# tictacmenthe/F2CNN

Measured on AMD Instinct MI355X. Metric: audio-seconds/sec through filterbank+envelope (HIP, 1 MI355X per rank); the +CNN figure of BASELINE's metric is value_with_cnn / blocks.cfg4, higher is better.
Workload: dtype f64 filter state + f64 utterance FFT + f32 row FFT; 1 GPU; cfg3: filterbank + Hilbert envelope + 50 Hz LPF in one call (f32 FFT), batch of 1000 x 1 s utterances per GPU, 128 channels, ENV1 (float64) out; channels=128, lpf_hz=50, launch_batch=1000, outputs_resident_in_hbm=True, parallelism=utterance-sharded x1, no collective, utterances_sent_back_by_the_accuracy_guard=0

## Files before the change

### f2cnn_amd/csrc/f2_api.hip

```cpp
#include "f2_internal.h"

char g_f2_err[512] = {0};

int f2_fail(f2_ctx* ctx, int code, const char* fmt, ...) {
    char* dst = ctx ? ctx->err : g_f2_err;
    va_list ap;
    va_start(ap, fmt);
    vsnprintf(dst, 512, fmt, ap);
    va_end(ap);
    return code;
}

int f2_reserve(f2_ctx* ctx, f2_scratch& s, size_t bytes) {
    if (bytes <= s.bytes) return F2_OK;
    if (s.ptr) {
        F2_HIP(ctx, hipStreamSynchronize(ctx->stream));
        F2_HIP(ctx, hipFree(s.ptr));
        s.ptr = nullptr;
        s.bytes = 0;
    }
    size_t want = (bytes + 255) & ~size_t(255);
    hipError_t e = hipMalloc(&s.ptr, want);
    if (e != hipSuccess) {
        s.ptr = nullptr;
// ... 220 lines not shown
    (void)hipStreamSynchronize(ctx->stream);
    f2_scratch* all[] = {&ctx->coefs, &ctx->offsets, &ctx->stage_in, &ctx->stage_out, &ctx->stage_aux,
                         &ctx->work,  &ctx->work2,   &ctx->xbuf,      &ctx->flags,    &ctx->gather_log, &ctx->dense_in,
                         &ctx->stamps, &ctx->noise_wave, &ctx->noise_meta, &ctx->acc_meta, &ctx->score_meta};
    for (f2_scratch* s : all)
        if (s->ptr) (void)hipFree(s->ptr);
    for (auto& v : ctx->prof)
        for (auto& pr : v) {
            (void)hipEventDestroy(pr.first);
            (void)hipEventDestroy(pr.second);
        }
    for (hipEvent_t e : ctx->prof_pool) (void)hipEventDestroy(e);
    for (auto& prec : ctx->tw)
        for (f2_scratch& s : prec)
            if (s.ptr) (void)hipFree(s.ptr);
    for (auto& prec : ctx->tw_large)
        for (f2_scratch& s : prec)
            if (s.ptr) (void)hipFree(s.ptr);
    for (f2_scratch& s : ctx->tw_p3)
        if (s.ptr) (void)hipFree(s.ptr);
    for (f2_scratch& s : ctx->tw_fl)
        if (s.ptr) (void)hipFree(s.ptr);
    for (f2_scratch& s : ctx->tw_split)
        if (s.ptr) (void)hipFree(s.ptr);
    for (f2_scratch* sc : {&ctx->tw_pair[0], &ctx->tw_pair[1], &ctx->pair_list[0], &ctx->pair_list[1]})
        if (sc->ptr) (void)hipFree(sc->ptr);
    if (ctx->work3.ptr) (void)hipFree(ctx->work3.ptr);
    if (ctx->k1_states.ptr) (void)hipFree(ctx->k1_states.ptr);
    if (ctx->k1_mtab.ptr) (void)hipFree(ctx->k1_mtab.ptr);
    if (ctx->k1_order.ptr) (void)hipFree(ctx->k1_order.ptr);
    if (ctx->handoff.ptr) (void)hipFree(ctx->handoff.ptr);
    if (ctx->handoff_off.ptr) (void)hipFree(ctx->handoff_off.ptr);
    for (auto& t : ctx->spec_tabs)
        for (f2_scratch* sc : {&t.hu, &t.e, &t.lgroup, &t.e64})
            if (sc->ptr) (void)hipFree(sc->ptr);
    for (f2_scratch* sc : {&ctx->spec_x, &ctx->spec_rho, &ctx->spec_xpart, &ctx->spec_meta, &ctx->spec_uflag, &ctx->spec_lptab})
        if (sc->ptr) (void)hipFree(sc->ptr);
    for (auto& prec : ctx->tw_sp)
        for (f2_scratch& sc : prec)
            if (sc.ptr) (void)hipFree(sc.ptr);
    for (auto& sp : ctx->up_inflight) (void)hipEventDestroy(sp.done);
    for (auto& b : ctx->up_big) {
        if (b.ptr) (void)hipHostFree(b.ptr);
        (void)hipEventDestroy(b.done);
    }
    if (ctx->up_ring) (void)hipHostFree(ctx->up_ring);
    if (ctx->host_flags) (void)hipHostFree(ctx->host_flags);
    if (ctx->own_stream && ctx->stream) (void)hipStreamDestroy(ctx->stream);
    delete ctx;
    return F2_OK;
}

int f2_ctx_synchronize(f2_ctx* ctx) {
    F2_CHECK(nullptr, ctx, F2_ERR_INVALID, "ctx is NULL");
    F2_HIP(ctx, hipStreamSynchronize(ctx->stream));
    return F2_OK;
}

int f2_ctx_set_stream(f2_ctx* ctx, void* hip_stream) {
    F2_CHECK(nullptr, ctx, F2_ERR_INVALID, "ctx is NULL");
    F2_HIP(ctx, hipStreamSynchronize(ctx->stream));
    if (ctx->own_stream && ctx->stream) F2_HIP(ctx, hipStreamDestroy(ctx->stream));
    if (hip_stream) {
        ctx->stream = (hipStream_t)hip_stream;
        ctx->own_stream = false;
    } else {
        F2_HIP(ctx, hipStreamCreateWithFlags(&ctx->stream, hipStreamNonBlocking));
        ctx->own_stream = true;
    }
// ... 523 lines not shown
```

### f2cnn_amd/csrc/f2_internal.h

```cpp
#pragma once
#include <hip/hip_runtime.h>

#include <cstdarg>
#include <cstdint>
#include <cstdio>
#include <cstring>
#include <mutex>
#include <string>
#include <utility>
#include <vector>

#include "../../include/f2cnn_hip.h"

struct f2_scratch {
    void* ptr = nullptr;
    size_t bytes = 0;
};

struct f2_spec_tables {
    int log2h = 0, C = 0;
    std::vector<double> coefs;
    int64_t tpitch = 0;
    f2_scratch hu, e, lgroup, e64;
};
#define F2_SPECTRAL_MIN_LOG2H 12
#define F2_SPECTRAL_MAX_LOG2H 15

struct f2_ctx {
    int device = 0;
    hipStream_t stream = nullptr;
    bool own_stream = true;
    int num_cus = 0;
    char err[512] = {0};
    f2_scratch coefs;
    f2_scratch offsets;
    f2_scratch stage_in;
    f2_scratch stage_out;
    f2_scratch stage_aux;
    f2_scratch work;
    f2_scratch work2;
    f2_scratch xbuf;
    f2_scratch dense_in;
    f2_scratch noise_wave;
    f2_scratch noise_meta;
    f2_scratch acc_meta;
    f2_scratch score_meta;
    f2_scratch gather_log;
    f2_scratch tw[2][16];
    f2_scratch tw_fl[16];
    f2_scratch tw_p3[2];
    f2_scratch tw_large[2][24];
    f2_scratch tw_split[24];
    std::vector<int> pair_list_host[2];
    f2_scratch tw_pair[2], pair_list[2];
    f2_scratch work3;
    f2_scratch handoff, handoff_off;
    std::vector<int64_t> handoff_off_host;
    f2_scratch k1_states, k1_mtab;
    f2_scratch k1_order;
    int k1_mtab_L = 0;
    std::vector<double> k1_mtab_coefs;
    std::vector<int64_t> offsets_host;
    std::vector<double> coefs_host;
    bool prof_on = false;
    struct prof_span {
        hipEvent_t first, second;
        bool closed;
    };
    std::vector<prof_span> prof[F2_K_COUNT];
    std::vector<hipEvent_t> prof_pool;
    std::vector<f2_spec_tables> spec_tabs;
    f2_scratch spec_x, spec_rho;
    f2_scratch spec_xpart;
    f2_scratch spec_meta, spec_uflag;
    f2_scratch spec_gdump;
    size_t spec_gdump_rows = 0;
    std::vector<int> spec_meta_host;
    int spec_coefs_ok = -1;
    int spec_min_pad = 64;
    size_t spec_last_B = 0;
    f2_scratch tw_sp[2][16];
    f2_scratch spec_lptab;
    double spec_lptab_a1 = 0.0;
    int spec_lptab_nt = 0;
    int opt_spectral = 1;
    int opt_spectral_min_rows = 4096;
    float opt_spectral_tol = 4e-6f;
    int opt_spectral_min_pad = -1;
    int opt_spectral_guard_dump = 0;
    int opt_k1_split = -1;
    int opt_k1_queue = -1;
    int opt_k1_qwaves = 0;
    int opt_env_pair = 1;
    int opt_cnn_f16x3 = 1;
    int opt_cnn_ws = 1;
    int opt_cnn_ws_dense = 1;
    int opt_gather_blocked = 1;
    int opt_env_plan4 = 0;
    char* up_ring = nullptr;
    size_t up_cap = 0, up_head = 0;
    struct up_span {
        size_t begin, end;
        hipEvent_t done;
    };
// ... 139 lines not shown
                             int nutt, int log2h, int C, int lpf, double b0, double a1, const float* d_x32,
                             const int64_t* d_x32_off, const int* d_uflag = nullptr);
bool f2_envelope_pair_supports(int log2h, int precision);
int f2_launch_envelope_pair(f2_ctx* ctx, const double* d_gfb, double* d_env, const int64_t* d_offsets,
                            const int64_t* h_offsets, const int* utts, int nutt, int log2h, int C, int lpf, double b0,
                            double a1, const float* d_x32, const int64_t* d_x32_off, const int64_t* h_x32_off,
                            const int* d_uflag = nullptr);
#define F2_MAX_LOG2M_LARGE 22
int f2_launch_envelope_large(f2_ctx* ctx, const double* d_x, double* d_y, int64_t n, int C, int lpf, double b0,
                             double a1, int precision);

static inline int f2_log2_ceil(int64_t n) {
    int k = 0;
    while ((int64_t(1) << k) < n) ++k;
    return k;
}

struct f2_handoff {
    bool f32 = false;
    float* d_x32 = nullptr;
    const int64_t* d_x32_off = nullptr;
    const int64_t* h_x32_off = nullptr;
};
int f2_plan_handoff(f2_ctx* ctx, const int64_t* h_offsets, int B, int C, int precision, bool want_gfb, f2_handoff* plan);
int f2_envelopes_device(f2_ctx* ctx, const void* d_wave, int wave_dtype, const int64_t* h_offsets, int B, int C, int lpf,
                        double cutoff_hz, int fft_precision, double* d_env, double* d_gfb, bool spectral);
int f2_launch_filterbank(f2_ctx* ctx, const void* d_wave, int wave_dtype, const int64_t* d_offsets,
                         const int64_t* h_offsets, const double* d_coefs, int B, int C, double* d_gfb,
                         const f2_handoff* handoff = nullptr, const int* d_uflag = nullptr, const int* h_flag0 = nullptr);
int f2_launch_envelope(f2_ctx* ctx, const double* d_gfb, const int64_t* d_offsets, const int64_t* h_offsets,
                       int B, int C, int lpf, double cutoff_hz, int precision, double* d_env,
                       const f2_handoff* handoff = nullptr, const int* d_uflag = nullptr, const int* h_flag0 = nullptr);
bool f2_spectral_supports_len(int64_t n, int min_pad);
bool f2_spectral_supports_coefs(const std::vector<double>& coefs, int C, std::vector<int>* Lgroup, int* min_pad);
int f2_launch_spectral(f2_ctx* ctx, const void* d_wave, int wave_dtype, const int64_t* d_offsets, const double* d_coefs,
                       int C, const int* d_ulist, int nutt, int64_t min_n , int log2h, int lpf,
                       double cutoff_hz, double* d_env, int* d_uflag);
int f2_launch_gather(f2_ctx* ctx, const double* d_env, int C, int64_t N, const int64_t* d_centers,
                     int64_t first_center, int64_t n_windows, int radius, int step, int normalize, float* d_out, int* d_flag);
int f2_launch_gather_ragged(f2_ctx* ctx, const double* d_env, int C, const int64_t* d_offsets, const int64_t* d_centers,
                            const int* d_win_utt, int64_t n_windows, int radius, int step, int normalize, float* d_out,
                            int* d_flag);
int f2_upload_windows(f2_ctx* ctx, const int64_t* centers, const int* win_utt, int64_t n_windows, const int64_t** d_centers,
                      const int** d_win_utt);
struct f2_win_seg {
    int utt;
    int64_t first, count;
};
int f2_launch_gather_strided(f2_ctx* ctx, const double* d_env, int C, const int64_t* d_offsets, const int64_t* h_offsets,
                             const f2_win_seg* segs, int nseg, int radius, int step, int hop, float* d_out, int* d_flag);
bool f2_gather_strided_blocked(const f2_ctx* ctx, int C, int step, int hop);
int64_t f2_gather_strided_columns(int64_t count, int radius, int step, int hop);
struct f2_cnn_route {
    bool split = false, ws = false, ws_dense = false;
};
f2_cnn_route f2_cnn_capability(const f2_cnn* cnn);
f2_cnn_route f2_cnn_call_route(const f2_ctx* ctx, const f2_cnn* cnn, bool have_scale_set);
bool f2_cnn_ws_supported(int rows, int channels);
bool f2_dense1_ws_takes(int K, int64_t n);
int f2_launch_dense1_ws(f2_ctx* ctx, const f2_cnn* cnn, const f2_scale_set* S, const float* a4, int64_t n, int K, float* a5);
int f2_launch_cnn_ws(f2_ctx* ctx, const f2_cnn* cnn, const f2_scale_set* S, const float* d_x, int64_t n, void* a2s, float* a4);
int f2_launch_cnn(f2_ctx* ctx, const f2_cnn* cnn, const f2_scale_set* S, f2_cnn_route route, const float* d_x, int64_t n, float* d_ws,
                  float* d_scores, uint8_t* d_labels);
int f2_launch_cnn_convs(f2_ctx* ctx, const f2_cnn* cnn, const f2_scale_set* S, f2_cnn_route route, const float* d_x, int64_t n,
                        float* d_ws, float* a4);
int f2_launch_cnn_dense(f2_ctx* ctx, const f2_cnn* cnn, const f2_scale_set* S, f2_cnn_route route, const float* a4, int64_t n, float* a5,
                        float* d_scores, uint8_t* d_labels);
// ... 17 lines not shown
```

### f2cnn_amd/csrc/f2_spectral.hip

```cpp
#define f2fft f2fft_sp
#undef F2_PLAN13_PASSES
#define F2_PLAN13_PASSES 4
#include <algorithm>
#include <cmath>
#include <complex>
#include <thread>

#include "f2_fft_lds.h"

using namespace f2fft;

namespace {

typedef float f2_f4 __attribute__((ext_vector_type(4)));
constexpr int SPEC_GB = 16;

constexpr int KS_CGROUP = 32;
constexpr int KS_CGROUP_LONG = 8;
constexpr int KS_STORE_AUX = 2;
typedef unsigned int f2_u4 __attribute__((ext_vector_type(4)));
typedef unsigned int f2_u2 __attribute__((ext_vector_type(2)));
__device__ __forceinline__ __amdgpu_buffer_rsrc_t row_buffer(double* y, int n) {
    return __builtin_amdgcn_make_buffer_rsrc(y, 0, n * 8, 0x00020000);
}
// ... 642 lines not shown
    if (tid == 0) {
        const cpx<double> z0 = lds[cpad(0)];
        if constexpr (LOGD == 0) {
            Xo[0] = {(float)(z0.re + z0.im), 0.f};
            Xo[H] = {(float)(z0.re - z0.im), 0.f};
        } else {
            Xp[0] = {z0.re + z0.im, 0.0};
            Xp[H] = {z0.re - z0.im, 0.0};
        }
    }
}

template <int LOG2HS, int LOGD>
__global__ __launch_bounds__(256) void k_spectrum_combine(const cpx<double>* __restrict__ Xpart, const cpx<double>* __restrict__ e64,
                                                          cpx<float>* __restrict__ X, int64_t xpitch) {
    constexpr int D = 1 << LOGD, HS = 1 << LOG2HS, H = D * HS, M = 2 * H;
    const int ul = blockIdx.y;
    const int k = blockIdx.x * 256 + threadIdx.x;
    if (k > H) return;
    const int kk = k & (2 * HS - 1);
    double re = 0.0, im = 0.0;
#pragma unroll
    for (int ph = 0; ph < D; ++ph) {
        const cpx<double>* __restrict__ Xp = Xpart + ((size_t)ul * D + ph) * (HS + 1);
        cpx<double> xp = kk <= HS ? Xp[kk] : Xp[2 * HS - kk];
        if (kk > HS) xp.im = -xp.im;
        const cpx<double> w = e64[(ph * k) & (M - 1)];
        re += xp.re * w.re - xp.im * w.im;
        im += xp.re * w.im + xp.im * w.re;
    }
    X[(size_t)ul * xpitch + k] = {(float)re, (float)im};
}

constexpr int TAIL_TB = 32;
constexpr int TAIL_WAVES = 4;

template <typename WaveT>
__global__ __launch_bounds__((64 * TAIL_WAVES)) void k_tail_state(const WaveT* __restrict__ wave, const int64_t* __restrict__ offsets,
                                                                const double* __restrict__ coefs, int C, int groups,
                                                                const int* __restrict__ ulist, int nutt,
                                                                const int* __restrict__ Lgroup, float* __restrict__ rho,
                                                                double two_over_m) {
    __shared__ double xss[TAIL_WAVES][TAIL_TB];
    const int lane = threadIdx.x & 63;
    const int wid = __builtin_amdgcn_readfirstlane(threadIdx.x >> 6);
    const int unit = blockIdx.x * TAIL_WAVES + wid;
    if (unit >= nutt * groups) return;
    const int ul = unit / groups, g = unit - ul * groups;
    const int b = ulist[ul];
    const int64_t off = offsets[b];
    const int64_t N = offsets[b + 1] - off;
    const int cc = g * 64 + lane;
    const int c = min(cc, C - 1);
    const double* k = coefs + (size_t)c * 10;
    const double rB0 = 1.0 / k[6];
    const double b0 = k[0] * rB0, a1 = k[7] * rB0, a2 = k[8] * rB0;
    const double c1 = k[1] / k[0], c2 = k[2] / k[0], c3 = k[3] / k[0], c4 = k[4] / k[0];
    const double scale = (b0 * b0) * (b0 * b0) / k[9] * two_over_m;
    double* xs = xss[wid];
    const WaveT* w = wave + off;
    const int64_t L = min((int64_t)Lgroup[g], N);
    const int64_t nblk = (L + TAIL_TB - 1) / TAIL_TB;
    const int64_t t_begin = N - nblk * TAIL_TB;
    double z10 = 0, z11 = 0, z20 = 0, z21 = 0, z30 = 0, z31 = 0, z40 = 0, z41 = 0;
    auto sample = [&](int64_t t) { return (lane < TAIL_TB && t >= 0 && t < N) ? (double)w[t] : 0.0; };
    double xnext = sample(t_begin + lane);
    for (int64_t t0 = t_begin; t0 < N; t0 += TAIL_TB) {
        if (lane < TAIL_TB) xs[lane] = xnext;
        xnext = sample(t0 + TAIL_TB + lane);
        __builtin_amdgcn_fence(__ATOMIC_RELEASE, "wavefront");
        __builtin_amdgcn_wave_barrier();
        __builtin_amdgcn_fence(__ATOMIC_ACQUIRE, "wavefront");
        double p1 = 0, p2 = 0, p3 = 0;
#pragma unroll
        for (int s2 = 0; s2 < TAIL_TB + 3; ++s2) {
            double n1 = 0, n2 = 0, n3 = 0;
            if (s2 < TAIL_TB) {
                const double wv = fma(-a1, z10, fma(-a2, z11, xs[s2]));
                n1 = fma(c1, z10, wv);
                z11 = z10;
                z10 = wv;
            }
            if (s2 >= 1 && s2 - 1 < TAIL_TB) {
                const double wv = fma(-a1, z20, fma(-a2, z21, p1));
                n2 = fma(c2, z20, wv);
                z21 = z20;
                z20 = wv;
            }
            if (s2 >= 2 && s2 - 2 < TAIL_TB) {
                const double wv = fma(-a1, z30, fma(-a2, z31, p2));
                n3 = fma(c3, z30, wv);
                z31 = z30;
                z30 = wv;
            }
            if (s2 >= 3) {
                const double wv = fma(-a1, z40, fma(-a2, z41, p3));
                z41 = z40;
                z40 = wv;
            }
            p1 = n1;
            p2 = n2;
            p3 = n3;
        }
        __builtin_amdgcn_fence(__ATOMIC_RELEASE, "wavefront");
        __builtin_amdgcn_wave_barrier();
        __builtin_amdgcn_fence(__ATOMIC_ACQUIRE, "wavefront");
    }
    const double ia2 = 1.0 / a2;
    const double R10 = (a1 - c1) * z10 + a2 * z11, R11 = a2 * z10 + c1 * a2 * z11;
    const double R20 = (a1 - c2) * z20 + a2 * z21, R21 = a2 * z20 + c2 * a2 * z21;
    const double R30 = (a1 - c3) * z30 + a2 * z31, R31 = a2 * z30 + c3 * a2 * z31;
    const double R40 = (a1 - c4) * z40 + a2 * z41, R41 = a2 * z40 + c4 * a2 * z41;
    double d0[2], d1[2], d2[2], d3[2];
    d3[0] = R40;
    d3[1] = R41;
    {
        const double p0 = R30, p1q = R31 + c4 * R30, p2q = c4 * R31;
        const double q = p2q * ia2;
        d2[0] = p0 - q;
        d2[1] = p1q - q * a1;
        d3[0] += q;
    }
    {
        const double s0 = 1.0, s1 = c4 + c3, s2 = c4 * c3;
        double p0 = s0 * R20, p1q = s0 * R21 + s1 * R20, p2q = s1 * R21 + s2 * R20, p3q = s2 * R21;
        const double q1 = p3q * ia2;
        p2q -= q1 * a1;
        p1q -= q1;
        const double q0 = p2q * ia2;
        p1q -= q0 * a1;
        p0 -= q0;
        d1[0] = p0;
        d1[1] = p1q;
        d2[0] += q0;
        d2[1] += q1;
    }
    {
        const double s0 = 1.0, s1 = c4 + c3, s2 = c4 * c3;
        const double t0 = s0, t1 = s1 + c2 * s0, t2 = s2 + c2 * s1, t3 = c2 * s2;
        double p0 = t0 * R10, p1q = t0 * R11 + t1 * R10, p2q = t1 * R11 + t2 * R10, p3q = t2 * R11 + t3 * R10, p4q = t3 * R11;
        const double q2 = p4q * ia2;
        p3q -= q2 * a1;
        p2q -= q2;
        const double q1 = p3q * ia2;
        p2q -= q1 * a1;
        p1q -= q1;
        const double q0 = p2q * ia2;
        p1q -= q0 * a1;
        p0 -= q0;
        d0[0] = p0;
        d0[1] = p1q;
        const double qq = q2 * ia2;
        d1[0] += q0 - qq;
        d1[1] += q1 - qq * a1;
        d2[0] += qq;
    }
    if (cc < C) {
        float* r = rho + ((size_t)ul * C + cc) * 8;
        typedef float f4 __attribute__((ext_vector_type(4)));
        *reinterpret_cast<f4*>(r) = f4{(float)(d0[0] * scale), (float)(d0[1] * scale), (float)(d1[0] * scale), (float)(d1[1] * scale)};
        *reinterpret_cast<f4*>(r + 4) = f4{(float)(d2[0] * scale), (float)(d2[1] * scale), (float)(d3[0] * scale), (float)(d3[1] * scale)};
    }
}

__global__ __launch_bounds__(256) void k_spectral_tables(const double* __restrict__ coefs, int C, int H, int64_t tpitch,
                                                         f2_f4* __restrict__ hu, cpx<float>* __restrict__ e,
                                                         cpx<double>* __restrict__ e64) {
    const int M = 2 * H;
    const int64_t q = (int64_t)blockIdx.x * 256 + threadIdx.x;
    const int c = blockIdx.y;
    double sn, cs;
    sincospi(2.0 * (double)q / (double)M, &sn, &cs);
    const double wr = cs, wi = -sn;
    if (c == C) {
        if (q < M) {
            e[q] = {(float)wr, (float)wi};
            if (e64) e64[q] = {wr, wi};
        }
        return;
    }
    if (q >= tpitch) return;
    f2_f4 out = {0.f, 0.f, 0.f, 0.f};
    if (q <= H) {
        const double* k = coefs + (size_t)c * 10;
        const double rB0 = 1.0 / k[6];
        const double b0 = k[0] * rB0, a1 = k[7] * rB0, a2 = k[8] * rB0;
        const double s = (b0 * b0) * (b0 * b0) / k[9] * (2.0 / M);
        const double w2r = wr * wr - wi * wi, w2i = 2.0 * wr * wi;
        const double dr = 1.0 + a1 * wr + a2 * w2r, di = a1 * wi + a2 * w2i;
        const double dn = 1.0 / (dr * dr + di * di);
        const double ur = dr * dn, ui = -di * dn;
        double hr = s, hi = 0.0;
#pragma unroll
        for (int m = 0; m < 4; ++m) {
            const double cm = k[1 + m] / k[0];
            const double nr = 1.0 + cm * wr, ni = cm * wi;
            const double tr = nr * ur - ni * ui, ti = nr * ui + ni * ur;
            const double xr = hr * tr - hi * ti, xi = hr * ti + hi * tr;
            hr = xr;
            hi = xi;
        }
        out = {(float)hr, (float)hi, (float)ur, (float)ui};
    }
    hu[(size_t)c * tpitch + q] = out;
}

int64_t ringing_length(double a1, double a2, double tol, int64_t limit) {
    if (!(a2 > 1e-3 && a2 < 1.0) || a1 * a1 >= 4.0 * a2) return 0;
    const double lr = 0.5 * std::log(a2);
    const double np = std::max(1.0, -3.0 / lr);
    const double target = std::log(tol) + 3.0 * std::log(np) + np * lr;
    double lo = np, hi = np;
    while (3.0 * std::log(hi) + hi * lr > target) {
        hi *= 2;
        if (hi > (double)limit) return 0;
    }
    for (int it = 0; it < 60; ++it) {
        const double mid = 0.5 * (lo + hi);
        if (3.0 * std::log(mid) + mid * lr > target) lo = mid;
        else hi = mid;
    }
    return (int64_t)std::ceil(hi) + 64;
}

}

bool f2_spectral_supports_len(int64_t n, int min_pad) {
    if (n < 2) return false;
    const int log2h = f2_log2_ceil(n) - 1;
    if (log2h < F2_SPECTRAL_MIN_LOG2H || log2h > F2_SPECTRAL_MAX_LOG2H) return false;
    return (int64_t(2) << log2h) - n >= std::max(64, min_pad);
}

bool f2_spectral_supports_coefs(const std::vector<double>& coefs, int C, std::vector<int>* Lgroup, int* min_pad) {
    if (coefs.size() != (size_t)C * 10 || C <= 0) return false;
    const int groups = (C + 63) / 64;
    if (Lgroup) Lgroup->assign((size_t)groups, 0);
    double peak = 0.0;
    for (int c = 0; c < C; ++c) {
        const double* k = &coefs[(size_t)c * 10];
        if (k[5] != 0.0 || k[0] == 0.0 || k[6] == 0.0 || k[9] == 0.0) return false;
        for (int q = 0; q < 10; ++q)
            if (!std::isfinite(k[q])) return false;
        const int64_t L = ringing_length(k[7] / k[6], k[8] / k[6], 1e-8, int64_t(1) << 17);
        if (L <= 0) return false;
        if (Lgroup) (*Lgroup)[(size_t)c / 64] = std::max((*Lgroup)[(size_t)c / 64], (int)L);
        peak = std::max(peak, 3.0 / (-0.5 * std::log(k[8] / k[6])));
    }
    if (min_pad) *min_pad = ((int)std::ceil(1.1 * peak) + 31) / 32 * 32;
    return true;
}

static int spectral_tables(f2_ctx* ctx, const double* d_coefs, int C, int log2h, f2_spec_tables** out) {
    for (auto& t : ctx->spec_tabs)
        if (t.log2h == log2h && t.C == C && t.coefs == ctx->coefs_host) {
            *out = &t;
            return F2_OK;
        }
    if (ctx->spec_tabs.size() >= 6) {
        F2_HIP(ctx, hipStreamSynchronize(ctx->stream));
        for (f2_scratch* s : {&ctx->spec_tabs.front().hu, &ctx->spec_tabs.front().e, &ctx->spec_tabs.front().lgroup,
                              &ctx->spec_tabs.front().e64})
            if (s->ptr) (void)hipFree(s->ptr);
        ctx->spec_tabs.erase(ctx->spec_tabs.begin());
    }
    f2_spec_tables t;
    t.log2h = log2h;
    t.C = C;
    t.coefs = ctx->coefs_host;
    std::vector<int> Lg;
    if (!f2_spectral_supports_coefs(t.coefs, C, &Lg, nullptr)) return f2_fail(ctx, F2_ERR_INVALID, "coefficient table not eligible");
    const int H = 1 << log2h, M = 2 * H;
    t.tpitch = H + 8;
    F2_TRY(f2_reserve(ctx, t.hu, sizeof(float) * 4 * (size_t)C * (size_t)t.tpitch));
    F2_TRY(f2_reserve(ctx, t.e, sizeof(float) * 2 * (size_t)M));
    F2_TRY(f2_reserve(ctx, t.lgroup, sizeof(int) * Lg.size()));
    if (log2h > 13) F2_TRY(f2_reserve(ctx, t.e64, sizeof(double) * 2 * (size_t)M));
    hipLaunchKernelGGL(k_spectral_tables, dim3((unsigned)((M + 255) / 256), (unsigned)(C + 1)), dim3(256), 0, ctx->stream, d_coefs, C, H,
                       t.tpitch, (f2_f4*)t.hu.ptr, (cpx<float>*)t.e.ptr, (cpx<double>*)t.e64.ptr);
    F2_HIP(ctx, hipGetLastError());
    F2_TRY(f2_upload_async(ctx, t.lgroup.ptr, Lg.data(), sizeof(int) * Lg.size()));
    ctx->spec_tabs.push_back(std::move(t));
    *out = &ctx->spec_tabs.back();
    return F2_OK;
}

static int lowpass_table(f2_ctx* ctx, double a1, double b0, int nt, int sp, LowpassConsts* K, const f2_f4** d_tab) {
    const long double q = -(long double)a1;
    K->qf = (float)q;
    K->b0f = (float)b0;
    K->g1 = (float)powl(q, sp);
    K->g2 = (float)powl(q, 2 * sp);
    K->g4 = (float)powl(q, 4 * sp);
    K->g8 = (float)powl(q, 8 * sp);
    K->gw = (double)powl(q, 64 * sp);
    K->gblk = (double)powl(q, sp * nt);
    f2_scratch& slot = ctx->spec_lptab;
    double& slot_a1 = ctx->spec_lptab_a1;
    *d_tab = (const f2_f4*)slot.ptr;
    constexpr int TMAX = 1024;
    if (slot.ptr && slot_a1 == a1) return F2_OK;
    std::vector<float> tab((size_t)TMAX * 4);
    for (int t = 0; t < TMAX; ++t) {
        const int lane = t & 63;
        tab[4 * (size_t)t] = (float)powl(q, sp * (lane + 1));
        tab[4 * (size_t)t + 1] = (float)powl(q, sp * t);
        tab[4 * (size_t)t + 2] = (float)powl(q, sp * ((lane & 15) + 1));
        tab[4 * (size_t)t + 3] = (float)powl(q, sp * ((lane & 31) + 1));
    }
    F2_TRY(f2_reserve(ctx, slot, sizeof(float) * tab.size()));
    F2_TRY(f2_upload_async(ctx, slot.ptr, tab.data(), sizeof(float) * tab.size()));
    slot_a1 = a1;
    *d_tab = (const f2_f4*)slot.ptr;
    return F2_OK;
}

template <typename WaveT, int LOG2H>
static int launch_group(f2_ctx* ctx, const WaveT* d_wave, const int64_t* d_offsets, const double* d_coefs, int C,
                        const int* d_ulist, int nutt, int64_t min_n, int lpf, double b0, double a1, double* d_env, int* d_uflag,
                        float tol, cpx<float>* d_X, float* d_rho) {
    constexpr int H = 1 << LOG2H, M = 2 * H;
    f2_spec_tables* tab = nullptr;
    F2_TRY(spectral_tables(ctx, d_coefs, C, LOG2H, &tab));
    constexpr int LOGD = LOG2H > 13 ? LOG2H - 13 : 0, LOG2HS = LOG2H - LOGD;
    constexpr int FFTLOG = LOG2H == 15 ? 14 : LOG2H;
    F2_TRY(ensure_twiddles<double>(ctx, LOG2HS, ctx->tw_sp[1][LOG2HS]));
    F2_TRY(ensure_twiddles<float>(ctx, FFTLOG, ctx->tw_sp[0][FFTLOG]));
    const int64_t xpitch = H + 8;
    const int groups = (C + 63) / 64;
    F2_TRY(f2_prof_begin(ctx, F2_K_SPECTRUM));
    cpx<double>* d_part = nullptr;
    if constexpr (LOGD > 0) {
        F2_TRY(f2_reserve(ctx, ctx->spec_xpart, sizeof(double) * 2 * ((size_t)(1 << LOG2HS) + 1) * (size_t)nutt << LOGD));
        d_part = (cpx<double>*)ctx->spec_xpart.ptr;
    }
    hipLaunchKernelGGL((k_utterance_spectrum<WaveT, LOG2HS, LOGD>), dim3((unsigned)nutt << LOGD), dim3(threads_for<double, LOG2HS>()),
                       0, ctx->stream, d_wave, d_offsets, d_ulist, d_X, xpitch, d_part,
                       (const cpx<double>*)ctx->tw_sp[1][LOG2HS].ptr);
    F2_HIP(ctx, hipGetLastError());
    if constexpr (LOGD > 0) {
        hipLaunchKernelGGL((k_spectrum_combine<LOG2HS, LOGD>), dim3((unsigned)((H + 256) / 256), (unsigned)nutt), dim3(256), 0,
                           ctx->stream, (const cpx<double>*)d_part, (const cpx<double>*)tab->e64.ptr, d_X, xpitch);
        F2_HIP(ctx, hipGetLastError());
    }
    F2_TRY(f2_prof_end(ctx, F2_K_SPECTRUM));
    F2_TRY(f2_prof_begin(ctx, F2_K_TAIL));
    const int units = nutt * groups;
    hipLaunchKernelGGL((k_tail_state<WaveT>), dim3((unsigned)((units + TAIL_WAVES - 1) / TAIL_WAVES)), dim3(64 * TAIL_WAVES), 0,
                       ctx->stream, d_wave, d_offsets, d_coefs, C, groups, d_ulist, nutt, (const int*)tab->lgroup.ptr, d_rho,
                       2.0 / M);
    F2_HIP(ctx, hipGetLastError());
    F2_TRY(f2_prof_end(ctx, F2_K_TAIL));
    SpecParams P;
    P.xpitch = xpitch;
    P.tpitch = tab->tpitch;
    P.env = d_env;
    P.uflag = d_uflag;
    P.C = C;
    P.nutt = nutt;
    P.lpf = lpf;
    const f2_f4* d_lptab = nullptr;
    F2_TRY(lowpass_table(ctx, a1, b0, threads_for<float, FFTLOG>(), 2, &P.lp, &d_lptab));
    P.tol = tol;
    P.gdump = ctx->opt_spectral_guard_dump ? (float*)ctx->spec_gdump.ptr : nullptr;
    P.stamps = nullptr;
#ifdef F2_STAMPS
    F2_TRY(f2_stamps_buffer(ctx, (size_t)nutt * C, 8, &P.stamps));
#endif
    F2_TRY(f2_prof_begin(ctx, F2_K_FUSED));
    if constexpr (LOG2H == 15)
        hipLaunchKernelGGL(k_spectral_envelope_long, dim3((unsigned)((size_t)nutt * C)), dim3(threads_for<float, FFTLOG>()), 0,
                           ctx->stream, P, (const cpx<float>*)d_X, (const f2_f4*)tab->hu.ptr, (const cpx<float>*)tab->e.ptr,
                           (const float*)d_rho, d_offsets, d_ulist, d_lptab, (const cpx<float>*)ctx->tw_sp[0][FFTLOG].ptr);
    else if (min_n >= 15 * (M / 16))
        hipLaunchKernelGGL((k_spectral_envelope<FFTLOG, true>), dim3((unsigned)((size_t)nutt * C)), dim3(threads_for<float, FFTLOG>()), 0,
                           ctx->stream, P, (const cpx<float>*)d_X, (const f2_f4*)tab->hu.ptr, (const cpx<float>*)tab->e.ptr,
                           (const float*)d_rho, d_offsets, d_ulist, d_lptab, (const cpx<float>*)ctx->tw_sp[0][FFTLOG].ptr);
    else
        hipLaunchKernelGGL((k_spectral_envelope<FFTLOG, false>), dim3((unsigned)((size_t)nutt * C)), dim3(threads_for<float, FFTLOG>()), 0,
                           ctx->stream, P, (const cpx<float>*)d_X, (const f2_f4*)tab->hu.ptr, (const cpx<float>*)tab->e.ptr,
                           (const float*)d_rho, d_offsets, d_ulist, d_lptab, (const cpx<float>*)ctx->tw_sp[0][FFTLOG].ptr);
    F2_HIP(ctx, hipGetLastError());
    F2_TRY(f2_prof_end(ctx, F2_K_FUSED));
// ... 39 lines not shown
```

Before: 203,800 audio-seconds/s.

## Compute spectral tail state as a matrix product with precomputed impulse-response table

The per-channel sequential IIR recurrence that computed each utterance's tail filter state is replaced by a linear map. The host precomputes, for each channel pair, the impulse-response contribution of each tail sample to the 8 state digits and uploads it as a table. The kernel then evaluates the tail state with f64 MFMA (16x16x4) over tiles of 64 utterances, using buffer loads into LDS and a cross-wave reduction. This removes the serial per-sample dependency chain and uses matrix units, at the cost of a cached table of up to 64 MB and of a fixed length cap that could change accuracy for slowly decaying channels.

After: 205,000 audio-seconds/s (median of 6 runs). No clear change (+0.6%).

```diff
diff --git a/f2cnn_amd/csrc/f2_api.hip b/f2cnn_amd/csrc/f2_api.hip
--- a/f2cnn_amd/csrc/f2_api.hip
+++ b/f2cnn_amd/csrc/f2_api.hip
@@ -276,9 +276,9 @@
     if (ctx->handoff.ptr) (void)hipFree(ctx->handoff.ptr);
     if (ctx->handoff_off.ptr) (void)hipFree(ctx->handoff_off.ptr);
     for (auto& t : ctx->spec_tabs)
-        for (f2_scratch* sc : {&t.hu, &t.e, &t.lgroup, &t.e64})
+        for (f2_scratch* sc : {&t.hu, &t.e, &t.e64})
             if (sc->ptr) (void)hipFree(sc->ptr);
-    for (f2_scratch* sc : {&ctx->spec_x, &ctx->spec_rho, &ctx->spec_xpart, &ctx->spec_meta, &ctx->spec_uflag, &ctx->spec_lptab})
+    for (f2_scratch* sc : {&ctx->spec_tail.g, &ctx->spec_tail.meta, &ctx->spec_x, &ctx->spec_rho, &ctx->spec_xpart, &ctx->spec_meta, &ctx->spec_uflag, &ctx->spec_lptab})
         if (sc->ptr) (void)hipFree(sc->ptr);
     for (auto& prec : ctx->tw_sp)
         for (f2_scratch& sc : prec)
diff --git a/f2cnn_amd/csrc/f2_internal.h b/f2cnn_amd/csrc/f2_internal.h
--- a/f2cnn_amd/csrc/f2_internal.h
+++ b/f2cnn_amd/csrc/f2_internal.h
@@ -21,7 +21,12 @@
     int log2h = 0, C = 0;
     std::vector<double> coefs;
     int64_t tpitch = 0;
-    f2_scratch hu, e, lgroup, e64;
+    f2_scratch hu, e, e64;
+};
+struct f2_tail_table {
+    int C = 0;
+    std::vector<double> coefs;
+    f2_scratch g, meta;
 };
 #define F2_SPECTRAL_MIN_LOG2H 12
 #define F2_SPECTRAL_MAX_LOG2H 15
@@ -70,6 +75,7 @@
     std::vector<prof_span> prof[F2_K_COUNT];
     std::vector<hipEvent_t> prof_pool;
     std::vector<f2_spec_tables> spec_tabs;
+    f2_tail_table spec_tail;
     f2_scratch spec_x, spec_rho;
     f2_scratch spec_xpart;
     f2_scratch spec_meta, spec_uflag;
@@ -275,7 +281,7 @@
                        int B, int C, int lpf, double cutoff_hz, int precision, double* d_env,
                        const f2_handoff* handoff = nullptr, const int* d_uflag = nullptr, const int* h_flag0 = nullptr);
 bool f2_spectral_supports_len(int64_t n, int min_pad);
-bool f2_spectral_supports_coefs(const std::vector<double>& coefs, int C, std::vector<int>* Lgroup, int* min_pad);
+bool f2_spectral_supports_coefs(const std::vector<double>& coefs, int C, std::vector<int>* Lchan, int* min_pad);
 int f2_launch_spectral(f2_ctx* ctx, const void* d_wave, int wave_dtype, const int64_t* d_offsets, const double* d_coefs,
                        int C, const int* d_ulist, int nutt, int64_t min_n , int log2h, int lpf,
                        double cutoff_hz, double* d_env, int* d_uflag);
diff --git a/f2cnn_amd/csrc/f2_spectral.hip b/f2cnn_amd/csrc/f2_spectral.hip
--- a/f2cnn_amd/csrc/f2_spectral.hip
+++ b/f2cnn_amd/csrc/f2_spectral.hip
@@ -698,80 +698,216 @@
     X[(size_t)ul * xpitch + k] = {(float)re, (float)im};
 }
 
-constexpr int TAIL_TB = 32;
 constexpr int TAIL_WAVES = 4;
+constexpr int TAIL_UNIT = 8;
+constexpr int TAIL_XP = 65;
+constexpr int64_t TAIL_LMAX = 65472;
+constexpr size_t TAIL_TABLE_CAP = size_t(64) << 20;
+typedef double f2_d4v __attribute__((ext_vector_type(4)));
+
+template <typename WaveT>
+struct tail_stage {
+    typedef double type;
+    typedef double raw;
+    static constexpr int TS = 32;
+    static __device__ __forceinline__ raw load(__amdgpu_buffer_rsrc_t r, int byte_off) {
+        return __builtin_bit_cast(double, __builtin_amdgcn_raw_buffer_load_b64(r, byte_off, 0, 0));
+    }
+};
+template <>
+struct tail_stage<int16_t> {
+    typedef float type;
+    typedef int16_t raw;
+    static constexpr int TS = 64;
+    static __device__ __forceinline__ raw load(__amdgpu_buffer_rsrc_t r, int byte_off) {
+        return (int16_t)__builtin_amdgcn_raw_buffer_load_b16(r, byte_off, 0, 0);
+    }
+};
 
 template <typename WaveT>
 __global__ __launch_bounds__((64 * TAIL_WAVES)) void k_tail_state(const WaveT* __restrict__ wave, const int64_t* __restrict__ offsets,
-                                                                const double* __restrict__ coefs, int C, int groups,
-                                                                const int* __restrict__ ulist, int nutt,
-                                                                const int* __restrict__ Lgroup, float* __restrict__ rho,
-                                                                double two_over_m) {
-    __shared__ double xss[TAIL_WAVES][TAIL_TB];
+                                                                const double* __restrict__ coefs, int C,
+                                                                const int* __restrict__ ulist, int nutt, int ntiles,
+                                                                const double* __restrict__ G, const int* __restrict__ gmeta,
+                                                                float* __restrict__ rho, double two_over_m) {
+    typedef tail_stage<WaveT> stage;
+    typedef typename stage::type StageT;
+    typedef double __attribute__((may_alias)) double_alias;
+    constexpr int TS = stage::TS;
+    static_assert(sizeof(StageT) * TS * TAIL_XP >= sizeof(double) * 16 * 64, "the partial sums reuse a wave's staging area");
+    static_assert(TAIL_WAVES == 4 && TAIL_UNIT % 8 == 0, "four rows per instruction, two instructions per round of the loop");
+    __shared__ __attribute__((aligned(16))) StageT xss[TAIL_WAVES][TS * TAIL_XP];
     const int lane = threadIdx.x & 63;
     const int wid = __builtin_amdgcn_readfirstlane(threadIdx.x >> 6);
-    const int unit = blockIdx.x * TAIL_WAVES + wid;
-    if (unit >= nutt * groups) return;
-    const int ul = unit / groups, g = unit - ul * groups;
-    const int b = ulist[ul];
-    const int64_t off = offsets[b];
-    const int64_t N = offsets[b + 1] - off;
-    const int cc = g * 64 + lane;
-    const int c = min(cc, C - 1);
-    const double* k = coefs + (size_t)c * 10;
-    const double rB0 = 1.0 / k[6];
-    const double b0 = k[0] * rB0, a1 = k[7] * rB0, a2 = k[8] * rB0;
-    const double c1 = k[1] / k[0], c2 = k[2] / k[0], c3 = k[3] / k[0], c4 = k[4] / k[0];
-    const double scale = (b0 * b0) * (b0 * b0) / k[9] * two_over_m;
-    double* xs = xss[wid];
-    const WaveT* w = wave + off;
-    const int64_t L = min((int64_t)Lgroup[g], N);
-    const int64_t nblk = (L + TAIL_TB - 1) / TAIL_TB;
-    const int64_t t_begin = N - nblk * TAIL_TB;
-    double z10 = 0, z11 = 0, z20 = 0, z21 = 0, z30 = 0, z31 = 0, z40 = 0, z41 = 0;
-    auto sample = [&](int64_t t) { return (lane < TAIL_TB && t >= 0 && t < N) ? (double)w[t] : 0.0; };
-    double xnext = sample(t_begin + lane);
-    for (int64_t t0 = t_begin; t0 < N; t0 += TAIL_TB) {
-        if (lane < TAIL_TB) xs[lane] = xnext;
-        xnext = sample(t0 + TAIL_TB + lane);
+    const int npairs = (C + 1) / 2;
+    const int p = npairs - 1 - (int)(blockIdx.x / (unsigned)ntiles);
+    const int u0 = (int)(blockIdx.x % (unsigned)ntiles) * 64;
+    const int per = gmeta[2 * p + 1] / TAIL_WAVES;
+    const int t_begin = wid * per;
+    const double* __restrict__ g = G + ((size_t)gmeta[2 * p] + (size_t)t_begin) * 16 + lane;
+    StageT* xs = xss[wid];
+    typename stage::raw xr[64];
+    unsigned base_lo, base_hi;
+    int nbytes;
+    {
+        const int b = ulist[min(u0 + lane, nutt - 1)];
+        const int64_t off = offsets[b];
+        const unsigned long long a = (unsigned long long)(wave + off);
+        base_lo = (unsigned)a;
+        base_hi = (unsigned)(a >> 32);
+        nbytes = u0 + lane < nutt ? (int)(offsets[b + 1] - off) * (int)sizeof(WaveT) : 0;
+    }
+    auto fetch = [&](int tb) {
+        const int tbytes = (tb + lane + 1) * (int)sizeof(WaveT);
+#pragma unroll
+        for (int j = 0; j < 64; ++j) {
+            const unsigned long long a = ((unsigned long long)(unsigned)__builtin_amdgcn_readlane((int)base_hi, j) << 32) |
+                                         (unsigned)__builtin_amdgcn_readlane((int)base_lo, j);
+            const int nb = __builtin_amdgcn_readlane(nbytes, j);
+            const __amdgpu_buffer_rsrc_t r = __builtin_amdgcn_make_buffer_rsrc((WaveT*)a, 0, nb, 0x00020000);
+            xr[j] = stage::load(r, nb - tbytes);
+        }
+    };
+    double bn[TS / 4];
+    auto fetch_rows = [&](int s) {
+        const int cnt = min(TS, per - s * TS);
+        const double* __restrict__ gs = g + (size_t)s * (TS * 16);
+#pragma unroll
+        for (int q = 0; q < TS / 4; q += 2) {
+            bn[q] = bn[q + 1] = 0.0;
+            if (4 * q < cnt) {
+                bn[q] = gs[q * 64];
+                bn[q + 1] = gs[(q + 1) * 64];
+            }
+        }
+    };
+    const f2_d4v zero = {0.0, 0.0, 0.0, 0.0};
+    const double first = lane < 16 ? 1.0 : 0.0, index = lane < 16 ? (double)lane : 0.0;
+    const f2_d4v rowv = __builtin_amdgcn_mfma_f64_16x16x4f64(index, first, zero, 0, 0, 0);
+    const f2_d4v colv = __builtin_amdgcn_mfma_f64_16x16x4f64(first, index, zero, 0, 0, 0);
+    f2_d4v acc[4] = {zero, zero, zero, zero};
+    const int xrow = (lane >> 4) * TAIL_XP + (lane & 15);
+    const int nblk = (per + TS - 1) / TS;
+    fetch(t_begin);
+    fetch_rows(0);
+    for (int s = 0; s < nblk; ++s) {
+        if (TS == 64 || lane < TS) {
+#pragma unroll
+            for (int j = 0; j < 64; ++j) xs[lane * TAIL_XP + j] = (StageT)xr[j];
+        }
+        double bc[TS / 4];
+#pragma unroll
+        for (int q = 0; q < TS / 4; ++q) {
+            bc[q] = bn[q];
+            asm volatile("" : "+v"(bc[q]));
+        }
         __builtin_amdgcn_fence(__ATOMIC_RELEASE, "wavefront");
         __builtin_amdgcn_wave_barrier();
         __builtin_amdgcn_fence(__ATOMIC_ACQUIRE, "wavefront");
-        double p1 = 0, p2 = 0, p3 = 0;
-#pragma unroll
-        for (int s2 = 0; s2 < TAIL_TB + 3; ++s2) {
-            double n1 = 0, n2 = 0, n3 = 0;
-            if (s2 < TAIL_TB) {
-                const double wv = fma(-a1, z10, fma(-a2, z11, xs[s2]));
-                n1 = fma(c1, z10, wv);
-                z11 = z10;
-                z10 = wv;
+        if (s + 1 < nblk) {
+            fetch(t_begin + (s + 1) * TS);
+            fetch_rows(s + 1);
+        }
+#pragma unroll
+        for (int q = 0; q < TS / 4; ++q)
+#pragma unroll
+            for (int m = 0; m < 4; ++m) {
+                const double a = (double)xs[4 * q * TAIL_XP + xrow + 16 * m];
+                acc[m] = __builtin_amdgcn_mfma_f64_16x16x4f64(a, bc[q], acc[m], 0, 0, 0);
             }
-            if (s2 >= 1 && s2 - 1 < TAIL_TB) {
-                const double wv = fma(-a1, z20, fma(-a2, z21, p1));
-                n2 = fma(c2, z20, wv);
-                z21 = z20;
-                z20 = wv;
-            }
-            if (s2 >= 2 && s2 - 2 < TAIL_TB) {
-                const double wv = fma(-a1, z30, fma(-a2, z31, p2));
-                n3 = fma(c3, z30, wv);
-                z31 = z30;
-                z30 = wv;
-            }
-            if (s2 >= 3) {
-                const double wv = fma(-a1, z40, fma(-a2, z41, p3));
-                z41 = z40;
-                z40 = wv;
-            }
-            p1 = n1;
-            p2 = n2;
-            p3 = n3;
-        }
         __builtin_amdgcn_fence(__ATOMIC_RELEASE, "wavefront");
         __builtin_amdgcn_wave_barrier();
         __builtin_amdgcn_fence(__ATOMIC_ACQUIRE, "wavefront");
     }
+    double_alias* red = reinterpret_cast<double_alias*>(xs);
+#pragma unroll
+    for (int r = 0; r < 4; ++r) {
+        const int row = (int)rowv[r] & 15, col = (int)colv[r] & 15;
+#pragma unroll
+        for (int m = 0; m < 4; ++m) red[col * 64 + 16 * m + row] = acc[m][r];
+    }
+    __syncthreads();
+    double sum[4] = {0.0, 0.0, 0.0, 0.0};
+#pragma unroll
+    for (int w = 0; w < TAIL_WAVES; ++w) {
+        const double_alias* rw = reinterpret_cast<const double_alias*>(xss[w]);
+#pragma unroll
+        for (int q = 0; q < 4; ++q) sum[q] += rw[(4 * wid + q) * 64 + lane];
+    }
+    const int c = 2 * p + (wid >> 1);
+    const int ul = u0 + lane;
+    if (ul < nutt && c < C) {
+        const double* k = coefs + (size_t)c * 10;
+        const double b0 = k[0] * (1.0 / k[6]);
+        const double scale = (b0 * b0) * (b0 * b0) / k[9] * two_over_m;
+        typedef float f4v __attribute__((ext_vector_type(4)));
+        *reinterpret_cast<f4v*>(rho + ((size_t)ul * C + c) * 8 + 4 * (wid & 1)) =
+            f4v{(float)(sum[0] * scale), (float)(sum[1] * scale), (float)(sum[2] * scale), (float)(sum[3] * scale)};
+    }
+}
+
+__global__ __launch_bounds__(256) void k_spectral_tables(const double* __restrict__ coefs, int C, int H, int64_t tpitch,
+                                                         f2_f4* __restrict__ hu, cpx<float>* __restrict__ e,
+                                                         cpx<double>* __restrict__ e64) {
+    const int M = 2 * H;
+    const int64_t q = (int64_t)blockIdx.x * 256 + threadIdx.x;
+    const int c = blockIdx.y;
+    double sn, cs;
+    sincospi(2.0 * (double)q / (double)M, &sn, &cs);
+    const double wr = cs, wi = -sn;
+    if (c == C) {
+        if (q < M) {
+            e[q] = {(float)wr, (float)wi};
+            if (e64) e64[q] = {wr, wi};
+        }
+        return;
+    }
+    if (q >= tpitch) return;
+    f2_f4 out = {0.f, 0.f, 0.f, 0.f};
+    if (q <= H) {
+        const double* k = coefs + (size_t)c * 10;
+        const double rB0 = 1.0 / k[6];
+        const double b0 = k[0] * rB0, a1 = k[7] * rB0, a2 = k[8] * rB0;
+        const double s = (b0 * b0) * (b0 * b0) / k[9] * (2.0 / M);
+        const double w2r = wr * wr - wi * wi, w2i = 2.0 * wr * wi;
+        const double dr = 1.0 + a1 * wr + a2 * w2r, di = a1 * wi + a2 * w2i;
+        const double dn = 1.0 / (dr * dr + di * di);
+        const double ur = dr * dn, ui = -di * dn;
+        double hr = s, hi = 0.0;
+#pragma unroll
+        for (int m = 0; m < 4; ++m) {
+            const double cm = k[1 + m] / k[0];
+            const double nr = 1.0 + cm * wr, ni = cm * wi;
+            const double tr = nr * ur - ni * ui, ti = nr * ui + ni * ur;
+            const double xr = hr * tr - hi * ti, xi = hr * ti + hi * tr;
+            hr = xr;
+            hi = xi;
+        }
+        out = {(float)hr, (float)hi, (float)ur, (float)ui};
+    }
+    hu[(size_t)c * tpitch + q] = out;
+}
+
+int64_t ringing_length(double a1, double a2, double tol, int64_t limit) {
+    if (!(a2 > 1e-3 && a2 < 1.0) || a1 * a1 >= 4.0 * a2) return 0;
+    const double lr = 0.5 * std::log(a2);
+    const double np = std::max(1.0, -3.0 / lr);
+    const double target = std::log(tol) + 3.0 * std::log(np) + np * lr;
+    double lo = np, hi = np;
+    while (3.0 * std::log(hi) + hi * lr > target) {
+        hi *= 2;
+        if (hi > (double)limit) return 0;
+    }
+    for (int it = 0; it < 60; ++it) {
+        const double mid = 0.5 * (lo + hi);
+        if (3.0 * std::log(mid) + mid * lr > target) lo = mid;
+        else hi = mid;
+    }
+    return (int64_t)std::ceil(hi) + 64;
+}
+
+void tail_digits(double a1, double a2, double c1, double c2, double c3, double c4, double z10, double z11, double z20,
+                 double z21, double z30, double z31, double z40, double z41, double* d) {
     const double ia2 = 1.0 / a2;
     const double R10 = (a1 - c1) * z10 + a2 * z11, R11 = a2 * z10 + c1 * a2 * z11;
     const double R20 = (a1 - c2) * z20 + a2 * z21, R21 = a2 * z20 + c2 * a2 * z21;
@@ -821,72 +957,50 @@
         d1[1] += q1 - qq * a1;
         d2[0] += qq;
     }
-    if (cc < C) {
-        float* r = rho + ((size_t)ul * C + cc) * 8;
-        typedef float f4 __attribute__((ext_vector_type(4)));
-        *reinterpret_cast<f4*>(r) = f4{(float)(d0[0] * scale), (float)(d0[1] * scale), (float)(d1[0] * scale), (float)(d1[1] * scale)};
-        *reinterpret_cast<f4*>(r + 4) = f4{(float)(d2[0] * scale), (float)(d2[1] * scale), (float)(d3[0] * scale), (float)(d3[1] * scale)};
-    }
-}
-
-__global__ __launch_bounds__(256) void k_spectral_tables(const double* __restrict__ coefs, int C, int H, int64_t tpitch,
-                                                         f2_f4* __restrict__ hu, cpx<float>* __restrict__ e,
-                                                         cpx<double>* __restrict__ e64) {
-    const int M = 2 * H;
-    const int64_t q = (int64_t)blockIdx.x * 256 + threadIdx.x;
-    const int c = blockIdx.y;
-    double sn, cs;
-    sincospi(2.0 * (double)q / (double)M, &sn, &cs);
-    const double wr = cs, wi = -sn;
-    if (c == C) {
-        if (q < M) {
-            e[q] = {(float)wr, (float)wi};
-            if (e64) e64[q] = {wr, wi};
-        }
-        return;
-    }
-    if (q >= tpitch) return;
-    f2_f4 out = {0.f, 0.f, 0.f, 0.f};
-    if (q <= H) {
-        const double* k = coefs + (size_t)c * 10;
+    d[0] = d0[0], d[1] = d0[1], d[2] = d1[0], d[3] = d1[1], d[4] = d2[0], d[5] = d2[1], d[6] = d3[0], d[7] = d3[1];
+}
+
+int64_t tail_rows(int64_t L) {
+    constexpr int64_t Q = TAIL_WAVES * TAIL_UNIT;
+    return (L + Q - 1) / Q * Q;
+}
+
+int tail_pair_length(const std::vector<int>& Lc, int p) {
+    const size_t c = 2 * (size_t)p;
+    return c + 1 < Lc.size() ? std::max(Lc[c], Lc[c + 1]) : Lc[c];
+}
+
+void tail_table_host(const std::vector<double>& coefs, int C, const std::vector<int>& Lc, std::vector<double>* G,
+                     std::vector<int>* meta) {
+    const int npairs = (C + 1) / 2;
+    meta->assign((size_t)2 * npairs, 0);
+    int64_t rows = 0;
+    for (int p = 0; p < npairs; ++p) {
+        (*meta)[2 * (size_t)p] = (int)rows;
+        (*meta)[2 * (size_t)p + 1] = (int)tail_rows(tail_pair_length(Lc, p));
+        rows += tail_rows(tail_pair_length(Lc, p));
+    }
+    G->assign((size_t)rows * 16, 0.0);
+    for (int c = 0; c < C; ++c) {
+        const double* k = &coefs[(size_t)c * 10];
         const double rB0 = 1.0 / k[6];
-        const double b0 = k[0] * rB0, a1 = k[7] * rB0, a2 = k[8] * rB0;
-        const double s = (b0 * b0) * (b0 * b0) / k[9] * (2.0 / M);
-        const double w2r = wr * wr - wi * wi, w2i = 2.0 * wr * wi;
-        const double dr = 1.0 + a1 * wr + a2 * w2r, di = a1 * wi + a2 * w2i;
-        const double dn = 1.0 / (dr * dr + di * di);
-        const double ur = dr * dn, ui = -di * dn;
-        double hr = s, hi = 0.0;
-#pragma unroll
-        for (int m = 0; m < 4; ++m) {
-            const double cm = k[1 + m] / k[0];
-            const double nr = 1.0 + cm * wr, ni = cm * wi;
-            const double tr = nr * ur - ni * ui, ti = nr * ui + ni * ur;
-            const double xr = hr * tr - hi * ti, xi = hr * ti + hi * tr;
-            hr = xr;
-            hi = xi;
-        }
-        out = {(float)hr, (float)hi, (float)ur, (float)ui};
-    }
-    hu[(size_t)c * tpitch + q] = out;
-}
-
-int64_t ringing_length(double a1, double a2, double tol, int64_t limit) {
-    if (!(a2 > 1e-3 && a2 < 1.0) || a1 * a1 >= 4.0 * a2) return 0;
-    const double lr = 0.5 * std::log(a2);
-    const double np = std::max(1.0, -3.0 / lr);
-    const double target = std::log(tol) + 3.0 * std::log(np) + np * lr;
-    double lo = np, hi = np;
-    while (3.0 * std::log(hi) + hi * lr > target) {
-        hi *= 2;
-        if (hi > (double)limit) return 0;
-    }
-    for (int it = 0; it < 60; ++it) {
-        const double mid = 0.5 * (lo + hi);
-        if (3.0 * std::log(mid) + mid * lr > target) lo = mid;
-        else hi = mid;
-    }
-    return (int64_t)std::ceil(hi) + 64;
+        const double a1 = k[7] * rB0, a2 = k[8] * rB0;
+        const double c1 = k[1] / k[0], c2 = k[2] / k[0], c3 = k[3] / k[0], c4 = k[4] / k[0];
+        double z10 = 0, z11 = 0, z20 = 0, z21 = 0, z30 = 0, z31 = 0, z40 = 0, z41 = 0;
+        double* g = G->data() + (size_t)(*meta)[2 * (size_t)(c / 2)] * 16 + 8 * (c & 1);
+        for (int t = 0; t < tail_pair_length(Lc, c / 2); ++t, g += 16) {
+            const double x = t == 0 ? 1.0 : 0.0;
+            const double w1 = std::fma(-a1, z10, std::fma(-a2, z11, x)), y1 = std::fma(c1, z10, w1);
+            z11 = z10, z10 = w1;
+            const double w2 = std::fma(-a1, z20, std::fma(-a2, z21, y1)), y2 = std::fma(c2, z20, w2);
+            z21 = z20, z20 = w2;
+            const double w3 = std::fma(-a1, z30, std::fma(-a2, z31, y2)), y3 = std::fma(c3, z30, w3);
+            z31 = z30, z30 = w3;
+            const double w4 = std::fma(-a1, z40, std::fma(-a2, z41, y3));
+            z41 = z40, z40 = w4;
+            tail_digits(a1, a2, c1, c2, c3, c4, z10, z11, z20, z21, z30, z31, z40, z41, g);
+        }
+    }
 }
 
 }
@@ -898,10 +1012,9 @@
     return (int64_t(2) << log2h) - n >= std::max(64, min_pad);
 }
 
-bool f2_spectral_supports_coefs(const std::vector<double>& coefs, int C, std::vector<int>* Lgroup, int* min_pad) {
+bool f2_spectral_supports_coefs(const std::vector<double>& coefs, int C, std::vector<int>* Lchan, int* min_pad) {
     if (coefs.size() != (size_t)C * 10 || C <= 0) return false;
-    const int groups = (C + 63) / 64;
-    if (Lgroup) Lgroup->assign((size_t)groups, 0);
+    std::vector<int> Lc((size_t)C, 0);
     double peak = 0.0;
     for (int c = 0; c < C; ++c) {
         const double* k = &coefs[(size_t)c * 10];
@@ -910,11 +1023,35 @@
             if (!std::isfinite(k[q])) return false;
         const int64_t L = ringing_length(k[7] / k[6], k[8] / k[6], 1e-8, int64_t(1) << 17);
         if (L <= 0) return false;
-        if (Lgroup) (*Lgroup)[(size_t)c / 64] = std::max((*Lgroup)[(size_t)c / 64], (int)L);
+        Lc[(size_t)c] = (int)std::min(L, TAIL_LMAX);
         peak = std::max(peak, 3.0 / (-0.5 * std::log(k[8] / k[6])));
     }
+    int64_t rows = 0;
+    for (int p = 0; p < (C + 1) / 2; ++p) rows += tail_rows(tail_pair_length(Lc, p));
+    if ((size_t)rows * 16 * sizeof(double) > TAIL_TABLE_CAP) return false;
+    if (Lchan) *Lchan = Lc;
     if (min_pad) *min_pad = ((int)std::ceil(1.1 * peak) + 31) / 32 * 32;
     return true;
+}
+
+static int tail_table(f2_ctx* ctx, int C, const double** d_G, const int** d_meta) {
+    f2_tail_table& t = ctx->spec_tail;
+    if (!(t.g.ptr && t.C == C && t.coefs == ctx->coefs_host)) {
+        std::vector<int> Lc, meta;
+        std::vector<double> G;
+        if (!f2_spectral_supports_coefs(ctx->coefs_host, C, &Lc, nullptr)) return f2_fail(ctx, F2_ERR_INVALID, "coefficient table not eligible");
+        tail_table_host(ctx->coefs_host, C, Lc, &G, &meta);
+        t.C = 0;
+        F2_TRY(f2_reserve(ctx, t.g, sizeof(double) * G.size()));
+        F2_TRY(f2_reserve(ctx, t.meta, sizeof(int) * meta.size()));
+        F2_TRY(f2_upload_async(ctx, t.g.ptr, G.data(), sizeof(double) * G.size()));
+        F2_TRY(f2_upload_async(ctx, t.meta.ptr, meta.data(), sizeof(int) * meta.size()));
+        t.coefs = ctx->coefs_host;
+        t.C = C;
+    }
+    *d_G = (const double*)t.g.ptr;
+    *d_meta = (const int*)t.meta.ptr;
+    return F2_OK;
 }
 
 static int spectral_tables(f2_ctx* ctx, const double* d_coefs, int C, int log2h, f2_spec_tables** out) {
@@ -925,8 +1062,7 @@
         }
     if (ctx->spec_tabs.size() >= 6) {
         F2_HIP(ctx, hipStreamSynchronize(ctx->stream));
-        for (f2_scratch* s : {&ctx->spec_tabs.front().hu, &ctx->spec_tabs.front().e, &ctx->spec_tabs.front().lgroup,
-                              &ctx->spec_tabs.front().e64})
+        for (f2_scratch* s : {&ctx->spec_tabs.front().hu, &ctx->spec_tabs.front().e, &ctx->spec_tabs.front().e64})
             if (s->ptr) (void)hipFree(s->ptr);
         ctx->spec_tabs.erase(ctx->spec_tabs.begin());
     }
@@ -934,18 +1070,15 @@
     t.log2h = log2h;
     t.C = C;
     t.coefs = ctx->coefs_host;
-    std::vector<int> Lg;
-    if (!f2_spectral_supports_coefs(t.coefs, C, &Lg, nullptr)) return f2_fail(ctx, F2_ERR_INVALID, "coefficient table not eligible");
+    if (!f2_spectral_supports_coefs(t.coefs, C, nullptr, nullptr)) return f2_fail(ctx, F2_ERR_INVALID, "coefficient table not eligible");
     const int H = 1 << log2h, M = 2 * H;
     t.tpitch = H + 8;
     F2_TRY(f2_reserve(ctx, t.hu, sizeof(float) * 4 * (size_t)C * (size_t)t.tpitch));
     F2_TRY(f2_reserve(ctx, t.e, sizeof(float) * 2 * (size_t)M));
-    F2_TRY(f2_reserve(ctx, t.lgroup, sizeof(int) * Lg.size()));
     if (log2h > 13) F2_TRY(f2_reserve(ctx, t.e64, sizeof(double) * 2 * (size_t)M));
     hipLaunchKernelGGL(k_spectral_tables, dim3((unsigned)((M + 255) / 256), (unsigned)(C + 1)), dim3(256), 0, ctx->stream, d_coefs, C, H,
                        t.tpitch, (f2_f4*)t.hu.ptr, (cpx<float>*)t.e.ptr, (cpx<double>*)t.e64.ptr);
     F2_HIP(ctx, hipGetLastError());
-    F2_TRY(f2_upload_async(ctx, t.lgroup.ptr, Lg.data(), sizeof(int) * Lg.size()));
     ctx->spec_tabs.push_back(std::move(t));
     *out = &ctx->spec_tabs.back();
     return F2_OK;
@@ -993,7 +1126,9 @@
     F2_TRY(ensure_twiddles<double>(ctx, LOG2HS, ctx->tw_sp[1][LOG2HS]));
     F2_TRY(ensure_twiddles<float>(ctx, FFTLOG, ctx->tw_sp[0][FFTLOG]));
     const int64_t xpitch = H + 8;
-    const int groups = (C + 63) / 64;
+    const double* d_G = nullptr;
+    const int* d_gmeta = nullptr;
+    F2_TRY(tail_table(ctx, C, &d_G, &d_gmeta));
     F2_TRY(f2_prof_begin(ctx, F2_K_SPECTRUM));
     cpx<double>* d_part = nullptr;
     if constexpr (LOGD > 0) {
@@ -1011,10 +1146,9 @@
     }
     F2_TRY(f2_prof_end(ctx, F2_K_SPECTRUM));
     F2_TRY(f2_prof_begin(ctx, F2_K_TAIL));
-    const int units = nutt * groups;
-    hipLaunchKernelGGL((k_tail_state<WaveT>), dim3((unsigned)((units + TAIL_WAVES - 1) / TAIL_WAVES)), dim3(64 * TAIL_WAVES), 0,
-                       ctx->stream, d_wave, d_offsets, d_coefs, C, groups, d_ulist, nutt, (const int*)tab->lgroup.ptr, d_rho,
-                       2.0 / M);
+    const int ntiles = (nutt + 63) / 64;
+    hipLaunchKernelGGL((k_tail_state<WaveT>), dim3((unsigned)((size_t)ntiles * ((C + 1) / 2))), dim3(64 * TAIL_WAVES), 0, ctx->stream, d_wave,
+                       d_offsets, d_coefs, C, d_ulist, nutt, ntiles, d_G, d_gmeta, d_rho, 2.0 / M);
     F2_HIP(ctx, hipGetLastError());
     F2_TRY(f2_prof_end(ctx, F2_K_TAIL));
     SpecParams P;
```
